# Benny44/QPALM

Hardware: AMD Instinct MI355X
Metric: QP solves/sec (batched random n=1000,m=2000); `value` = solve only, batch resident in HBM -- with qpalm_setup in the clock as the reference's run_time has it: `value_setup_plus_solve` (higher is better)
Workload: dtype f64

## Files before the change

qpalm_amd/csrc/qpalm_capi.inc:

```
#include <math.h>
#include <stdio.h>
#include <stdlib.h>
#include <string.h>
#include <sys/mman.h>

#include <algorithm>
#include <atomic>
#include <chrono>
#include <thread>
#include <string>
#include <vector>
#include <map>

#include "../../include/qpalm_gfx950.h"

#ifdef QP_TWO_INSTANCES
#define QP_INST(ns, kern) ns::kern
#else
#define QP_INST(ns, kern) kern
#define QP_T_SMALL QP_T
#define QP_LDS_SMALL 38912
#define QP_T_TINY QP_T
#define QP_LDS_TINY 22016
#define QP_TINY_PER_CU 7
// ... 39 lines not shown
  if (s->eps_abs_in < 0 || s->eps_rel_in < 0 || (s->eps_rel_in == 0 && s->eps_abs_in == 0)) return 0;
  if (s->rho <= 0 || s->rho >= 1) return 0;
  if (s->eps_prim_inf < 0 || s->eps_dual_inf < 0) return 0;
  if (s->theta > 1 || s->delta <= 1 || s->sigma_max <= 0) return 0;
  if (s->proximal != 0 && s->proximal != 1) return 0;
  if (s->gamma_init <= 0 || s->gamma_upd < 1 || s->gamma_max < s->gamma_init) return 0;
  if (s->scaling < 0) return 0;
  if (s->warm_start != 0 && s->warm_start != 1) return 0;
  if (s->verbose != 0 && s->verbose != 1) return 0;
  if (s->print_iter <= 0 || s->reset_newton_iter <= 0) return 0;
  if (s->enable_dual_termination != 0 && s->enable_dual_termination != 1) return 0;
  return 1;
}

static size_t align_up(size_t v, size_t a) { return (v + a - 1) / a * a; }

struct qpg_ctx {
  int device;
  int lds_bytes;
  int max_slots;
  int update_rank_threshold;
  int narrow_rows;
  int place_panel_wave;
  int small_workgroups;
  int coop;
  int coop_workgroups;
  int coop_max_batch;
  int coop_rank_threshold;
  int queue_order;
  int coop_test_kill;
  int coop_graphs;
  int coop_updates;
  int sweep_ranks;
  int factor_fused_solve;
  int kkt_compact;
  int sequential_rank_sums;
  int linesearch_hbm;
  int sparse_gpw;
  int sparse_lds;
  int sparse_ordering;
  int sparse_factor;
  int sparse_coop;
  int sparse_kkt;
  int ld_align;
  void *mv_buf[5];
  size_t mv_cap[5];
};

enum { H_AP, H_AI, H_ATP, H_ATI, H_ATPERM, H_AINV, H_QP, H_QI, H_QFP, H_QFI, H_QFPERM, H_AX, H_QX, H_Q, H_BMIN, H_BMAX, H_COUNT };
struct HostProblem {
  int n, m, nzA, nzQ, nzQf;
  double c;
  bool set;
};

struct qpg_batch {
  qpg_ctx *ctx;
  int B, n, m, nnzA, nnzQ, nnzQf, ld, nslots, ls_stride;
  int small, threads, lds_bytes;
  int kkt, nfac;
  QPGSettings settings;
  std::vector<HostProblem> probs;
  char *hslab; size_t hslab_bytes, hoff[H_COUNT + 1], hper[H_COUNT], helem[H_COUNT];
  template <class T> T *harr(int a, size_t b) const { return (T *)(hslab + hoff[a]) + b * hper[a]; }
  std::thread arena_thread; int arena_rc; bool arena_clean;
  std::vector<int> host_status;
// ... 10 lines not shown
  std::vector<SpPlan> sp_plan;
  qpg_view V;
  bool is_setup;
  float last_solve_ms;
  std::vector<std::pair<std::string, std::pair<void *, size_t> > > named;
  struct CoGraph { int uses; bool ready; rt_graph_t exec; };
  std::map<int, CoGraph> co_graphs;
  std::string co_sig;
  long co_replays;
  long co_sweeps;
  int nnzA_in, nnzQ_in;
  std::vector<std::vector<int> > map_A, map_Q;
  void *val_maps_d = nullptr; bool val_maps_current = false;
  std::vector<double> raw_h;
  void *raw_d = nullptr; int raw_cur = 0;
  double sens_floor = 0.0;
  double *raw_q() { return raw_h.data(); }
  double *raw_bmin() { return raw_h.data() + (size_t)B * n; }
  double *raw_bmax() { return raw_h.data() + (size_t)B * n + (size_t)B * m; }
  double *raw_d_q() const { return (double *)raw_d; }
  double *raw_d_bmin() const { return (double *)raw_d + (size_t)B * n; }
  double *raw_d_bmax() const { return (double *)raw_d + (size_t)B * n + (size_t)B * m; }
};
static void co_graphs_clear(qpg_batch *bt) {
  for (auto &g : bt->co_graphs) if (g.second.ready) RT_GRAPH_FREE(g.second.exec);
  bt->co_graphs.clear();
}

extern "C" int qpg_ctx_create(int device, qpg_ctx **out) {
  if (!out) return fail(QPG_ERR_INVALID, "qpg_ctx_create: out is NULL");
  std::string why;
  if (RT_DEVICE_INIT(device, why) != 0) return fail(QPG_ERR_NO_DEVICE, "qpg_ctx_create: " + why);
  qpg_ctx *c = new qpg_ctx();
  c->device = device; c->lds_bytes = QPG_LDS_DEFAULT; c->max_slots = 512; c->update_rank_threshold = -1; c->small_workgroups = 1; c->place_panel_wave = 0; c->narrow_rows = 1; c->coop = -1; c->coop_workgroups = 256; c->coop_max_batch = 4; c->coop_rank_threshold = -2; c->coop_updates = 2; c->coop_test_kill = 0; c->queue_order = 1; c->coop_graphs = 1; c->ld_align = 16; c->sweep_ranks = 16; c->kkt_compact = 1; c->factor_fused_solve = 1; c->sparse_factor = -1; c->sparse_kkt = 0; c->sparse_coop = 0; c->sparse_ordering = -1; c->sparse_lds = 1; c->sparse_gpw = 0; c->linesearch_hbm = 0; c->sequential_rank_sums = -1;
  for (int k = 0; k < 5; k++) { c->mv_buf[k] = nullptr; c->mv_cap[k] = 0; }
  *out = c;
  return api_ok();
}
extern "C" void qpg_ctx_destroy(qpg_ctx *ctx) {
  if (!ctx) return;
  for (int k = 0; k < 5; k++) if (ctx->mv_buf[k]) RT_FREE(ctx->mv_buf[k]);
  RT_RELEASE_STREAMS();
  delete ctx;
}
static int ctx_scratch(qpg_ctx *ctx, int k, size_t bytes, void **p) {
  if (bytes > ctx->mv_cap[k]) {
    if (ctx->mv_buf[k]) RT_FREE(ctx->mv_buf[k]);
    ctx->mv_buf[k] = nullptr; ctx->mv_cap[k] = 0;
    const size_t cap = align_up(bytes + bytes / 2, 4096);
    if (RT_MALLOC(&ctx->mv_buf[k], cap) != 0) return 1;
    ctx->mv_cap[k] = cap;
  }
  *p = ctx->mv_buf[k];
  return 0;
}
extern "C" int qpg_ctx_set_option(qpg_ctx *ctx, const char *name, qpg_int value) {
  if (!ctx || !name) return fail(QPG_ERR_INVALID, "qpg_ctx_set_option: NULL");
  if (!strcmp(name, "lds_bytes")) { if (value < QPG_LDS_DEFAULT || value > 160 * 1024 - 8192) return fail(QPG_ERR_INVALID, "lds_bytes out of range"); ctx->lds_bytes = (int)value; }
  else if (!strcmp(name, "max_slots")) { if (value < 1) return fail(QPG_ERR_INVALID, "max_slots < 1"); ctx->max_slots = (int)value; }
  else if (!strcmp(name, "update_rank_threshold")) ctx->update_rank_threshold = (int)value;
  else if (!strcmp(name, "small_workgroups")) ctx->small_workgroups = (value >= 0 && value <= 3) ? (int)value : 1;
  else if (!strcmp(name, "place_panel_wave")) ctx->place_panel_wave = (value < 0 || value > 2) ? 2 : (int)value;
  else if (!strcmp(name, "narrow_rows")) ctx->narrow_rows = value ? 1 : 0;
  else if (!strcmp(name, "coop")) ctx->coop = (value < 0) ? -1 : (value ? 1 : 0);
  else if (!strcmp(name, "coop_rank_threshold")) ctx->coop_rank_threshold = (value < -1) ? -2 : (int)value;
  else if (!strcmp(name, "coop_updates")) ctx->coop_updates = (value >= 0 && value <= 2) ? (int)value : 2;
  else if (!strcmp(name, "coop_graphs")) ctx->coop_graphs = value ? 1 : 0;
  else if (!strcmp(name, "coop_test_kill")) ctx->coop_test_kill = (int)value;
  else if (!strcmp(name, "queue_order")) ctx->queue_order = value ? 1 : 0;
  else if (!strcmp(name, "sweep_ranks")) { if (value != 16 && value != 32) return fail(QPG_ERR_INVALID, "sweep_ranks must be 16 or 32"); ctx->sweep_ranks = (int)value; }
  else if (!strcmp(name, "kkt_compact")) ctx->kkt_compact = value ? 1 : 0;
  else if (!strcmp(name, "factor_fused_solve")) ctx->factor_fused_solve = value ? 1 : 0;
  else if (!strcmp(name, "sparse_factor")) ctx->sparse_factor = (value < 0) ? -1 : (value ? 1 : 0);
  else if (!strcmp(name, "sparse_kkt")) ctx->sparse_kkt = value ? 1 : 0;
  else if (!strcmp(name, "sparse_coop")) { if (value != 0 && value != 1) return fail(QPG_ERR_INVALID, "sparse_coop must be 0 or 1"); ctx->sparse_coop = (int)value; }
  else if (!strcmp(name, "sequential_rank_sums")) ctx->sequential_rank_sums = (value < 0) ? -1 : (value ? 1 : 0);
  else if (!strcmp(name, "linesearch_hbm")) ctx->linesearch_hbm = (value < 0) ? 0 : (int)std::min<qpg_int>(value, 1 << 20);
  else if (!strcmp(name, "sparse_gpw")) ctx->sparse_gpw = (int)value;
  else if (!strcmp(name, "sparse_lds")) ctx->sparse_lds = (value < 0) ? 0 : (int)value;
  else if (!strcmp(name, "sparse_ordering")) ctx->sparse_ordering = (value < 0) ? -1 : (value ? 1 : 0);
  else if (!strcmp(name, "ld_align")) { if (value != 8 && value != 16 && value != 32) return fail(QPG_ERR_INVALID, "ld_align must be 8, 16 or 32"); ctx->ld_align = (int)value; }
  else if (!strcmp(name, "coop_max_batch")) { if (value < 1) return fail(QPG_ERR_INVALID, "coop_max_batch < 1"); ctx->coop_max_batch = (int)value; }
  else if (!strcmp(name, "coop_workgroups")) { if (value < 1 || value > 4096) return fail(QPG_ERR_INVALID, "coop_workgroups out of range"); ctx->coop_workgroups = (int)value; }
  else return fail(QPG_ERR_INVALID, std::string("unknown option ") + name);
  return api_ok();
}

static int arena_alloc(qpg_batch *bt);
static void *host_slab_alloc(size_t bytes) {
  void *p = mmap(nullptr, std::max<size_t>(bytes, 4096), PROT_READ | PROT_WRITE, MAP_PRIVATE | MAP_ANONYMOUS, -1, 0);
  if (p == MAP_FAILED) return nullptr;
#ifdef MADV_HUGEPAGE
  if (bytes >= ((size_t)64 << 20)) (void)madvise(p, bytes, MADV_HUGEPAGE);
#endif
  return p;
}
static void host_slab_free(void *p, size_t bytes) { if (p) munmap(p, std::max<size_t>(bytes, 4096)); }

extern "C" int qpg_batch_create(qpg_ctx *ctx, qpg_int B, qpg_int n, qpg_int m, qpg_int nnzA_max, qpg_int nnzQ_max,
                                const QPGSettings *settings, qpg_batch **out) {
  if (!ctx || !out) return fail(QPG_ERR_INVALID, "qpg_batch_create: NULL argument");
  if (B <= 0 || n <= 0 || m < 0 || nnzA_max < 0 || nnzQ_max < 0) return fail(QPG_ERR_INVALID, "qpg_batch_create: bad dimensions");
  if (!qpg_validate_settings(settings)) return fail(QPG_ERR_INVALID, "Settings validation returned failure");
// ... 696 lines not shown
  RT_MEMCPY_H2D(V.d, x0.data(), x0.size() * sizeof(double));
  BT_LAUNCH(bt, k_lobpcg, blocks_for(bt), 0, V);
  if (RT_SYNC() != 0) return fail(QPG_ERR_RUNTIME, "k_lobpcg failed: " + std::string(RT_LAST_ERROR()));
  return QPG_OK;
}

extern "C" int qpg_batch_setup(qpg_batch *bt) {
  if (!bt) return fail(QPG_ERR_INVALID, "qpg_batch_setup: NULL");
  for (int b = 0; b < bt->B; b++) if (!bt->probs[b].set) return fail(QPG_ERR_INVALID, "qpg_batch_setup: problem not set for every batch member");
  co_graphs_clear(bt);
  qpg_view &V = bt->V;
  if (bt->arena_thread.joinable()) bt->arena_thread.join();
  if (bt->arena_rc != 0 || !bt->arena_d) return fail(QPG_ERR_ALLOC, "device allocation failed");
  if (!bt->arena_clean) {
    RT_MEMSET(bt->arena_d, 0, bt->arena_d_bytes);
    if (RT_SYNC() != 0) return fail(QPG_ERR_RUNTIME, "arena clear failed: " + std::string(RT_LAST_ERROR()));
  }
  bt->arena_clean = false;
  bt->is_setup = false;
  bt->raw_h.clear(); bt->raw_cur = 0;
  bt->val_maps_current = false;
  V.B = bt->B; V.n = bt->n; V.m = bt->m; V.ld = bt->ld; V.nnzA = bt->nnzA; V.nnzQ = bt->nnzQ; V.nnzQf = bt->nnzQf;
  V.ls_hbm = bt->ctx->linesearch_hbm; V.seq_mode = bt->ctx->sequential_rank_sums;
  V.nslots = bt->nslots; V.lds_bytes = bt->lds_bytes; V.update_rank_threshold = bt->ctx->update_rank_threshold; V.place_panel_wave = bt->ctx->place_panel_wave;
  V.ls_stride = bt->ls_stride;
  {
    size_t nnz_rows = 0, rows = 0;
    for (auto &hp : bt->probs) { nnz_rows += (size_t)hp.nzA; rows += (size_t)hp.m; }
    const size_t colbufs = (size_t)4 * (bt->threads / 64) * bt->n * sizeof(double);
    V.narrow_rows = (bt->ctx->narrow_rows && !bt->kkt && colbufs <= (size_t)bt->lds_bytes && nnz_rows <= 16 * std::max<size_t>(rows, 1)) ? 1 : 0;
  }
  V.wst_stride = (int)QPG_WST_STRIDE(bt->nfac);
  V.sweep_ranks = bt->ctx->sweep_ranks;
  V.kkt_compact = bt->ctx->kkt_compact;
  V.factor_fused_solve = bt->ctx->factor_fused_solve;
  V.kkt = bt->kkt; V.nfac = bt->nfac;
  if (ensure_dual_slots(bt) != 0) return fail(QPG_ERR_ALLOC, "device allocation failed (LD_Q slots)");
  V.sparse = 0; V.sp_co_G = 0; V.sp_co_wv = nullptr;
  bt->sp_plan.clear();
  if (bt->sparse) {
    const int rcs = sparse_setup(bt);
    if (rcs != QPG_OK) return rcs;
    if (ensure_dual_slots(bt) != 0) return fail(QPG_ERR_ALLOC, "device allocation failed (LD_Q values of the sparse factor)");
  }
  const size_t B = bt->B, n = bt->n, m = bt->m;
  {
    char *const dev[H_COUNT] = {(char *)V.Ap, (char *)V.Ai, (char *)V.Atp, (char *)V.Ati, (char *)V.Atperm, (char *)V.Ainv, (char *)V.Qp, (char *)V.Qi,
                                (char *)V.Qfp, (char *)V.Qfi, (char *)V.Qfperm, (char *)V.Ax, (char *)V.Qx, (char *)V.q, (char *)V.bmin, (char *)V.bmax};
    for (int a = 0; a < H_COUNT; a++)
      if (bt->hper[a] && RT_MEMCPY_H2D_ASYNC(dev[a], bt->hslab + bt->hoff[a], B * bt->hper[a] * bt->helem[a], 0) != 0)
        return fail(QPG_ERR_RUNTIME, "upload failed: " + std::string(RT_LAST_ERROR()));
    RT_COPY_MARK(0);
    std::vector<double> c0(B);
    std::vector<qpg_scalars> sc(B);
    const qpg_scalars sc0 = setup_scalars(bt);
    for (size_t b = 0; b < B; b++) {
      c0[b] = bt->probs[b].c; sc[b] = sc0; bt->host_status[b] = QPG_UNSOLVED;
      const int *Qp = bt->harr<int>(H_QP, b), *Qi = bt->harr<int>(H_QI, b);
      const double *Qx = bt->harr<double>(H_QX, b);
      int hint = 0;
      for (int j = 0; j < bt->probs[b].n && !hint; j++) {
        bool pos = false;
        for (int k = Qp[j]; k < Qp[j + 1]; k++) if (Qi[k] == j && Qx[k] > 0.0) { pos = true; break; }
        if (!pos) hint = 1;
      }
      sc[b].seq_hint = hint;
// ... 1130 lines not shown
```

qpalm_amd/csrc/qpalm_dense.h:

```cpp
#ifndef QPALM_DENSE_H
#define QPALM_DENSE_H
#include <type_traits>

#ifdef QPALM_EMU
#define QP_FLAG_LOAD(p) (*(volatile int *)(p))
#define QP_FLAG_STORE(p, v) (*(volatile int *)(p) = (v))
#define QP_RELEASE_AGENT() do { } while (0)
#define QP_ACQUIRE_AGENT() do { } while (0)
#define QP_DRAIN_VMEM() do { } while (0)
#define QP_SLEEP() do { } while (0)
#define QP_WAVE_SYNC() emu_wave_sync()
#define QP_LDS_VBASE(p) (p)
#define QP_SCHED_BARRIER() do { } while (0)
#define QP_SETPRIO(p) do { } while (0)
#define QP_DRAIN_LDS() do { } while (0)
#else
#define QP_FLAG_LOAD(p) __hip_atomic_load((p), __ATOMIC_RELAXED, __HIP_MEMORY_SCOPE_AGENT)
#define QP_FLAG_STORE(p, v) __hip_atomic_store((p), (v), __ATOMIC_RELAXED, __HIP_MEMORY_SCOPE_AGENT)
#define QP_RELEASE_AGENT() __builtin_amdgcn_fence(__ATOMIC_RELEASE, "agent")
#define QP_ACQUIRE_AGENT() __builtin_amdgcn_fence(__ATOMIC_ACQUIRE, "agent")
#define QP_DRAIN_VMEM() asm volatile("s_waitcnt vmcnt(0)" ::: "memory")
#define QP_SLEEP() __builtin_amdgcn_s_sleep(2)
#define QP_SETPRIO(p) __builtin_amdgcn_s_setprio(p)
#define QP_DRAIN_LDS() asm volatile("s_waitcnt lgkmcnt(0)" ::: "memory")
// ... 953 lines not shown
  dnew = qp_rank_pivots_seq<KG>(p, ln, d0);
  const double sh = qp_row_shr<1>(dnew);
  dprev = ((ln & 15) == 0) ? d0 : sh;
  return (mode != QP_PIV_SEQ) ? 1 : 0;
}

#ifdef QPALM_EMU
template <int K, int OFF, int R0, int R1>
QPD void qp_apply_ranks_dpp(const double cw0, const double cw1, double (&wrow)[K], double &l) {
  const int lane = threadIdx.x & 63;
  emu_publish2(cw0, cw1);
  for (int r = R0; r < R1 && OFF + r < K; r++) {
    const double c0 = emu_peek((lane & ~15) | r, 0), c1 = emu_peek((lane & ~15) | r, 1);
    wrow[OFF + r] = QP_FMA(c0, l, wrow[OFF + r]);
    l = QP_FMA(c1, wrow[OFF + r], l);
  }
  emu_wave_sync();
}
#else
#define QP_FD_STEP(i, n) "v_fmac_f64_dpp %" #i ", %9, %8 row_newbcast:%" #n " row_mask:0xf bank_mask:0xf bound_ctrl:1\n\t" \
                         "v_fmac_f64_dpp %8, %10, %" #i " row_newbcast:%" #n " row_mask:0xf bank_mask:0xf bound_ctrl:1\n\t"
#define QP_FD_EIGHT QP_FD_STEP(0, 11) QP_FD_STEP(1, 12) QP_FD_STEP(2, 13) QP_FD_STEP(3, 14) QP_FD_STEP(4, 15) QP_FD_STEP(5, 16) QP_FD_STEP(6, 17) QP_FD_STEP(7, 18)
template <int R0> QPD void qp_fmac_bcast8(double *w, double &l, const double cw0, const double cw1) {
  asm("s_nop 1\n\t" QP_FD_EIGHT
      : "+&v"(w[0]), "+&v"(w[1]), "+&v"(w[2]), "+&v"(w[3]), "+&v"(w[4]), "+&v"(w[5]), "+&v"(w[6]), "+&v"(w[7]), "+&v"(l)
      : "v"(cw0), "v"(cw1), "n"(R0), "n"(R0 + 1), "n"(R0 + 2), "n"(R0 + 3), "n"(R0 + 4), "n"(R0 + 5), "n"(R0 + 6), "n"(R0 + 7));
}
template <int K, int OFF, int R0, int R1>
QPD void qp_apply_ranks_dpp(const double cw0, const double cw1, double (&wrow)[K], double &l) {
  static_assert(R1 - R0 == 8 && K % 8 == 0, "eight ranks at a time");
  if constexpr (OFF + R1 <= K) qp_fmac_bcast8<R0>(&wrow[OFF + R0], l, cw0, cw1);
}
#endif
#ifndef QP_AQD
#define QP_AQD 4
#endif

template <class IP, class DP, class WP>
QPD int updown_scatter_rows(const IP Atp, const IP Ati, const DP Atss, const int n, const WP Wst, const IP cols,
                            const int n_up, const IP cols_dn, const int r0, const int kk, const int lane, const int wid) {
  int jmin = n;
  for (int r = wid; r < kk; r += QP_NW) {
    const int g = r0 + r;
    const int t = (g < n_up) ? cols[g] : cols_dn[g - n_up];
    for (int k = Atp[t] + lane; k < Atp[t + 1]; k += 64) {
      const int i = Ati[k];
      Wst[(size_t)r * n + i] = Atss[k];
      jmin = (i < jmin) ? i : jmin;
    }
  }
  return jmin;
}

template <int RPT, int K>
QPNI void dense_updown(const int *Atp_, const int *Ati_, const double *Atss_, const int n_, const int ld_,
                       double *L_, double *Dg_, double *Wst_, const int *cols_, int n_up_,
                       const int *cols_dn_, int n_dn_, QpShared *S_, char *lds, int64_t *tdbg_, int pre_jmin_ = -1,
                       double *fs_ = nullptr, int rk0_ = 0, int rkn_ = 0x7fffffff) {
  const int n = QP_UNIFORM(n_), ld = QP_UNIFORM(ld_), n_up = QP_UNIFORM(n_up_), n_dn = QP_UNIFORM(n_dn_);
  const int rk0 = QP_UNIFORM(rk0_), rkn = QP_UNIFORM(rkn_);
  const int pre_jmin = QP_UNIFORM(pre_jmin_);
  const int pivmode = QP_UNIFORM(S_->seq_ranks);
  qp_gdouble *fs = (qp_gdouble *)fs_;
  const bool fuse_any = QP_UNIFORM((int)(fs_ != nullptr)) != 0;
  int64_t QP_LDS_AS *tdbg = (int64_t QP_LDS_AS *)tdbg_;
  const qp_gint *Atp = (const qp_gint *)Atp_, *Ati = (const qp_gint *)Ati_, *cols = (const qp_gint *)cols_, *cols_dn = (const qp_gint *)cols_dn_;
  const qp_gdouble *Atss = (const qp_gdouble *)Atss_;
  qp_gdouble *L = (qp_gdouble *)L_, *Dg = (qp_gdouble *)Dg_, *Wst = (qp_gdouble *)Wst_;
  QpShared &S = *S_;
  static_assert(K == 8 || K == 16 || K == 32, "rank groups of one DPP row (16 lanes), eight ranks at a time");
  static_assert(K <= QPG_KWST, "the staging area holds QPG_KWST dense update vectors");
  typedef UpdownLds<RPT, K> UpdownLdsT;
  UpdownLdsT QP_LDS_AS &U = *QP_LDS_ARG(UpdownLdsT, lds);
  static_assert(sizeof(UpdownLds<RPT, K>) <= ((RPT == 1) ? QP_LDS_BUDGET : QPG_LDS_DEFAULT), "update scratch must fit the dynamic LDS (the 256-thread instance only ever runs RPT = 1)");
  constexpr int NB = UpdownCfg<K>::NB, G = UpdownCfg<K>::G, KG = UpdownCfg<K>::KG;
  constexpr int PROWS = QP_T * RPT;
  constexpr bool MP = (K > 16);
  static_assert(PROWS % NB == 0, "passes start on block boundaries");
  const int lane = threadIdx.x & 63, wid = QP_UNIFORM(S.wave_rank[threadIdx.x >> 6]), tid = wid * 64 + lane;
  const int nr_all = n_up + n_dn;
  const int rk1 = (rkn < nr_all - rk0) ? (rk0 + rkn) : nr_all;
  qp_gdouble *dummy = Wst + (size_t)QPG_KWST * n;
  qp_gdouble *Tab = dummy + QPG_DUMMY + QPG_HSTASH;
  const int npass = MP ? (n + PROWS - 1) / PROWS : 1;
  for (int r0 = rk0; r0 < rk1; r0 += K) {
    const int kk = (rk1 - r0 < K) ? (rk1 - r0) : K;
    const bool fuse = fuse_any && (r0 + K >= nr_all);
    __syncthreads();
    long long tq0 = QP_CLOCK();
    int jmin = n;
    if (pre_jmin < 0) {
      for (int e = tid; e < kk * n; e += QP_T) Wst[e] = 0.0;
      __syncthreads();
      jmin = updown_scatter_rows(Atp, Ati, Atss, n, Wst, cols, n_up, cols_dn, r0, kk, lane, wid);
    } else jmin = (pre_jmin < n) ? pre_jmin : n - 1;
    if (fuse) jmin = 0;
    jmin = QP_UNIFORM(block_imin(S, jmin));
    double ialpha[G], sg[G];
    const int rl = lane & 15;
#pragma unroll
    for (int g = 0; g < G; g++) {
      ialpha[g] = 1.0;
      sg[g] = (16 * g + rl < kk) ? ((r0 + 16 * g + rl < n_up) ? 1.0 : -1.0) : 0.0;
    }
    const int J0 = (jmin / NB) * NB;
    if (tid == 0) {
      const long long tq1 = QP_CLOCK(); tdbg[0] += tq1 - tq0; tq0 = tq1;
      tdbg[QPG_CNT_SWEEPS] += 1;
      tdbg[QPG_CNT_SWEEP_ENTRIES] += (long long)(n - J0) * (n - J0 - 1) / 2 + (n - J0);
    }
    for (int pass = 0; pass < npass; pass++) {
    const int R0 = pass * PROWS;
    const int R1 = (!MP || n - R0 < PROWS) ? n : R0 + PROWS;
    const int Js = (J0 > R0) ? J0 : R0;
    if (Js >= R1) continue;
    const bool last_pass = (R1 >= n);
    const int rlim = last_pass ? ld : R1;
    if (MP && npass > 1) __syncthreads();
    double w[RPT][K];
#pragma unroll
// ... 156 lines not shown
      const bool own_live0 = (R0 + 64 * RPT - 1 >= Ja);
      auto owner_block = [&]() QP_ALWAYS_INLINE {
        const long long tt0 = QP_CLOCK();
        bool any = false;
#pragma unroll
        for (int rr = 0; rr < RPT; rr++) { const int i = R0 + tid * RPT + rr; any = any || (i >= Ja && i < R1); }
        constexpr bool WAVES = MP;
        if (s > 0 && (WAVES ? (__ballot(any ? 1 : 0) != 0ull) : any)) {
          const int i0 = R0 + tid * RPT;
          apply_table(prv, Jp, i0 >= Ja && i0 < rlim);
        }
#pragma unroll
        for (int rr = 0; rr < RPT; rr++) {
          const int i = R0 + tid * RPT + rr;
          if (i >= Jn && i < Jn + jbn) {
#pragma unroll
            for (int r = 0; r < K; r++) U.Wd[prv][i - Jn][r] = w[rr][r];
            U.Wd[prv][i - Jn][K] = acc[rr];
          }
        }
        if (wid == 0) {
#pragma unroll
          for (int rr = 0; rr < RPT; rr++)
#pragma unroll
            for (int r = 0; r < K; r++) U.stash[rr][r][lane] = w[rr][r];
#pragma unroll
          for (int rr = 0; rr < RPT; rr++) U.stash_acc[rr][lane] = acc[rr];
        }
        if (tid == QP_T - 64) tdbg[2] += QP_CLOCK() - tt0;
      };
      if (wid == 0) {
        const long long tp0 = QP_CLOCK();
        QP_SETPRIO(3);
        double wrow[K];
        double accp;
#pragma unroll
        for (int r = 0; r < K; r++) wrow[r] = (lane < jb) ? U.Wd[cur][lane][r] : 0.0;
        accp = (lane < jb) ? U.Wd[cur][lane][K] : 0.0;
        if (s > 0) {
          constexpr bool PSQ = QP_USQ;
          constexpr int QD = PSQ ? QP_AQD : 8;
          qp_gdouble *rowp = (lane < jb) ? (L + (size_t)Jp * ld + J + lane) : (dummy + lane);
          const size_t cstride = (lane < jb) ? (size_t)ld : 0;
          const int lrow = lane & (NB - 1);
          double q[QD];
#pragma unroll
          for (int cc = 0; cc < QD; cc++) q[cc] = PSQ ? U.Lsq[cur][cc][lrow] : rowp[(size_t)cc * cstride];
          const qp_pair QP_LDS_AS *tabA = (const qp_pair QP_LDS_AS *)QP_LDS_VBASE(&QP_CWG(U, prv, 0)[lane & 15][0]);
          constexpr bool PADPP = (K <= 16);
          qp_pair cfq[PADPP ? QD : 1][G];
          if (PADPP) {
#pragma unroll
            for (int cc = 0; cc < QD; cc++)
#pragma unroll
              for (int g = 0; g < G; g++) cfq[cc][g] = tabA[cc * K + 16 * g];
          }
          auto group = [&](const int c0) QP_ALWAYS_INLINE {
#pragma unroll
            for (int u = 0; u < QD; u++) {
              const int c1 = c0 + u;
              double l = q[u];
              const int cpre = (c1 + QD < NB) ? c1 + QD : NB - 1;
              if (PADPP) {
                qp_apply_ranks_dpp<K, 0, 0, 8>(cfq[u][0].x, cfq[u][0].y, wrow, l);
                if (KG > 8 && kk > 8) qp_apply_ranks_dpp<K, 0, 8, 16>(cfq[u][0].x, cfq[u][0].y, wrow, l);
                if constexpr (G > 1) {
// ... 62 lines not shown
              nwv[g] = 0.0; ngam[g] = 0.0;
              if (g > 0 && kkg <= 0) continue;
              const double wv = (rk < kkg) ? wt[(16 * g + rk) & (K - 1)] : 0.0;
              if (QP_PANEL_TIMING == 2 && g == 0) { QP_DRAIN_LDS(); const long long t = QP_CLOCK(); if (lane == 0) tdbg[8] += t - tc0; tc0 = t; }
              const double p = sg[g] * wv * wv * ialpha[g];
              double dnew, dprev;
              if (qp_rank_pivots<KG>(p, ln, d0, pivmode, dnew, dprev) && lane == 0) tdbg[QPG_CNT_SEQ_COLS] += 1;
              const double rdn = qp_rcp(dnew);
              const double gam = -sg[g] * wv * ialpha[g] * rdn;
              if (ln < KG) { QP_CWG(U, cur, c1)[16 * g + ln][0] = -wv; QP_CWG(U, cur, c1)[16 * g + ln][1] = -gam; }
              ialpha[g] = (wv == 0.0) ? ialpha[g] : ialpha[g] * dprev * rdn;
              d0 = qp_readlane(dnew, kkg - 1);
              nwv[g] = -wv; ngam[g] = -gam;
            }
            if (QP_PANEL_TIMING == 2) { double gg = ngam[0]; QP_OPAQUE_V(gg); const long long t = QP_CLOCK(); if (lane == 0) tdbg[9] += t - tc0; tc0 = t; }
            if (ln == c1) dreg = d0;
            double l = lcur;
            qp_apply_ranks_dpp<K, 0, 0, 8>(nwv[0], ngam[0], wrow, l);
            if (KG > 8 && kk > 8) qp_apply_ranks_dpp<K, 0, 8, 16>(nwv[0], ngam[0], wrow, l);
            if constexpr (G > 1) {
              if (kk > 16) qp_apply_ranks_dpp<K, 16, 0, 8>(nwv[1], ngam[1], wrow, l);
              if (kk > 24) qp_apply_ranks_dpp<K, 16, 8, 16>(nwv[1], ngam[1], wrow, l);
            }
            const bool below = (ln > c1 && ln < jb);
            if (below) U.Ld[cur][ln][c1] = l;
            if constexpr (FS) { const double yc = qp_readlane(vsub, c1); vsub = QP_FMA(-(below ? l : 0.0), yc, vsub); }
            if (QP_PANEL_TIMING == 2) { double ll = l; QP_OPAQUE_V(ll); const long long t = QP_CLOCK(); if (lane == 0) tdbg[11] += t - tc0; }
            QP_SCHED_BARRIER();
          }
        };
        if constexpr (FOLD) { if (fuse) recurrence(std::true_type()); else recurrence(std::false_type()); }
        else recurrence(std::false_type());
        if (QP_PANEL_TIMING == 1 && lane == 0) tdbg[9] += QP_CLOCK() - tp1;
        const long long tp2 = QP_CLOCK();
        if constexpr (!FOLD) if (fuse) {
          double lc = (lane > 0 && lane < jb) ? U.Ld[cur][lane][0] : 0.0;
#pragma unroll 1
          for (int c = 0; c < jb; c++) {
            const int ln = QP_FRESH_LANE(lane);
            const double lcn = (ln > c + 1 && ln < jb) ? U.Ld[cur][ln][c + 1] : 0.0;
            const double yc = qp_readlane(vsub, c);
            vsub = QP_FMA(-lc, yc, vsub);
            lc = lcn;
          }
        }
        if (fuse && lane < jb) { U.ys[cur][lane] = vsub; fs[J + lane] = vsub; }
        if (lane < jb) Dg[J + lane] = dreg;
        if (!QP_USQ) {
#pragma unroll 1
          for (int c = 0; c < jb; c++)
            if (lane > c && lane < jb) L[(size_t)(J + c) * ld + (J + lane)] = U.Ld[cur][lane][c];
        }
#pragma unroll
        for (int rr = 0; rr < RPT; rr++)
#pragma unroll
          for (int r = 0; r < K; r++) w[rr][r] = own_live0 ? U.stash[rr][r][lane] : 0.0;
#pragma unroll
        for (int rr = 0; rr < RPT; rr++) acc[rr] = own_live0 ? U.stash_acc[rr][lane] : 0.0;
        QP_SETPRIO(0);
        if (lane == 0) { tdbg[1] += QP_CLOCK() - tp0; tdbg[QPG_CNT_SWEEP_COLS] += jb; }
        if (QP_PANEL_TIMING == 1 && lane == 0) tdbg[10] += QP_CLOCK() - tp2;
        tpe = QP_CLOCK();
      }
      if (wid != 0 || own_live0) owner_block();
      constexpr int NFREE = (QP_NW == 1) ? 0 : 1;
      if (wid >= NFREE) {
        const int t0 = tid - 64 * NFREE, nt = QP_T - 64 * NFREE;
        if (QP_USQ) {
          for (int e = t0; e < NB * NB; e += nt) {
            const int c1 = e / NB, c = e % NB;
            if (c > c1) {
              if (s > 0) L[(size_t)(Jp + c1) * ld + (Jp + c)] = U.Ld[prv][c][c1];
              if (c < jbn) U.Ld[prv][c][c1] = L[(size_t)(Jn + c1) * ld + (Jn + c)];
            }
            if (jbn > 0) U.Lsq[prv][c1][c] = (c < jbn) ? L[(size_t)(J + c1) * ld + (Jn + c)] : 0.0;
          }
        } else {
          for (int e = t0; e < jbn * jbn; e += nt) {
            const int c1 = e / jbn, c = e % jbn;
            if (c > c1) U.Ld[prv][c][c1] = L[(size_t)(Jn + c1) * ld + (Jn + c)];
          }
        }
        if (t0 < jbn) U.dd[prv][t0] = Dg[Jn + t0];
        if (MP && !last_pass && s > 0) export_table(prv, Jp, t0, nt);
// ... 367 lines not shown
```

qpalm_amd/csrc/qpalm_device.h:

```cpp
#ifndef QPALM_DEVICE_H
#define QPALM_DEVICE_H

#include "qpalm_types.h"

#ifndef QP_T
#define QP_T 512
#endif
#define QP_NW (QP_T / 64)
#ifndef QP_KSEL
#define QP_KSEL(RPT) ((RPT) <= 2 ? 16 : 8)
#endif
#ifndef QP_K32
#ifdef QPALM_EMU
#define QP_K32(RPT) ((RPT) >= 1 && (RPT) <= 2)
#define QP_LDS_BUDGET QPG_LDS_DEFAULT
#else
#define QP_K32(RPT) (QP_T >= 512 && (RPT) >= 1 && (RPT) <= 2)
#define QP_LDS_BUDGET ((QP_T >= 512) ? QPG_LDS_DEFAULT : 38912)
#endif
#endif
#define QPD __device__ __forceinline__
#define QPN __device__ __forceinline__
#ifndef QP_PHASE_CALLS
#define QP_PHASE_CALLS 2
// ... 75 lines not shown
}
#define QP_FRESH_LANE(lane) qp_fresh_lane_()
static __device__ __forceinline__ int qp_fresh_tid_() {
  int t = (int)threadIdx.x;
  asm volatile("" : "+v"(t));
  return t & 1023;
}
#define QP_FRESH_TID() qp_fresh_tid_()
static __device__ __forceinline__ int qp_opaque_true_() {
  int one;
  asm volatile("s_mov_b32 %0, 1" : "=s"(one));
  return one;
}
#define QP_CALL_BLOCK() qp_opaque_true_()
#define QP_ALWAYS_INLINE __attribute__((always_inline))
#define QP_HW_SIMD() ((int)__builtin_amdgcn_s_getreg((2 - 1) << 11 | 4 << 6 | 4))
#define QP_HW_CU_KEY() ((int)(__builtin_amdgcn_s_getreg((8 - 1) << 11 | 8 << 6 | 4) | (__builtin_amdgcn_s_getreg((4 - 1) << 11 | 0 << 6 | 20) << 8)))
#endif

QPD double qmax(double a, double b) { return (a > b) ? a : b; }
QPD double qmin(double a, double b) { return (a < b) ? a : b; }
QPD double qabs(double x) { return (x < 0) ? -x : x; }

#define QP_NRED 20
struct QpShared {
  double red[QP_NW][QP_NRED];
  double bc[QP_NRED];
  int    ired[QP_NW][4];
  int    ibc[8];
  int    hw_simd[QP_NW];
  int    placement;
  int    panel_wave;
  int    seq_ranks;
  int    wave_rank[QP_NW];
};

#define QP_PIV_TREE 0
#define QP_PIV_SEQ 1
#define QP_PIV_GUARD 2
QPD int qp_pivot_mode(const qpg_view &V, int b) {
  if (V.seq_mode > 0 || (V.seq_mode < 0 && (V.sc[b].nc_flag != 0 || V.sc[b].seq_hint != 0))) return QP_PIV_SEQ;
  return (V.seq_mode < 0) ? QP_PIV_GUARD : QP_PIV_TREE;
}

QPD double wave_sum(double v) {
  for (int o = 32; o > 0; o >>= 1) v += __shfl_xor(v, o);
  return v;
}
QPD double wave_max(double v) {
  for (int o = 32; o > 0; o >>= 1) { double u = __shfl_xor(v, o); v = (u > v) ? u : v; }
  return v;
}
QPD int wave_isum(int v) {
  for (int o = 32; o > 0; o >>= 1) v += __shfl_xor(v, o);
  return v;
}
QPD int wave_imax(int v) {
  for (int o = 32; o > 0; o >>= 1) { int u = __shfl_xor(v, o); v = (u > v) ? u : v; }
  return v;
}
QPD int wave_imin(int v) {
  for (int o = 32; o > 0; o >>= 1) { int u = __shfl_xor(v, o); v = (u < v) ? u : v; }
  return v;
}

template <int NM, int NS>
// ... 148 lines not shown
```

qpalm_amd/csrc/qpalm_iter.h:

```cpp
#ifndef QPALM_ITER_H
#define QPALM_ITER_H
#ifndef QP_NOFUSE
#define QP_NOFUSE 0
#endif

#define QP_KIND_NEWTON 0
#define QP_KIND_OUTER 1
#define QP_KIND_FORCED 2
#define QP_KIND_TERMINATED 3

QPD int qp_prox(const qpg_settings &st, const qpg_scalars &s) { return (st.proximal != 0 || s.nc_flag != 0) ? 1 : 0; }
QPD double qp_gamma_init(const qpg_settings &st, const qpg_scalars &s) { return s.nc_flag ? s.nc_gamma : st.gamma_init; }
QPD double qp_gamma_max(const qpg_settings &st, const qpg_scalars &s) { return s.nc_flag ? s.nc_gamma : st.gamma_max; }

struct IterShared {
  QpShared S;
  qpg_scalars s;
  int kind, action, nL, pos;
  double a0, b0;
  double scan_a[QP_NW], scan_b[QP_NW];
};

struct QpArrays {
  const qpg_view *V; int b, n, m;
// ... 176 lines not shown
    }
  } else {
    for (int i = tid; i < m; i += QP_T) a.y()[i] = 0.;
  }
  __syncthreads();
  double vm[1] = {0.0}, vs[3] = {0.0, 0.0, 0.0};
  for (int j = tid; j < n; j += QP_T) { vs[0] += a.x()[j] * a.Qxv()[j]; vs[1] += a.q()[j] * a.x()[j]; }
  for (int i = tid; i < m; i += QP_T) {
    const double ax = a.Axv()[i];
    const double mid = qmax(a.bmin()[i], qmin(ax, a.bmax()[i]));
    const double t = ax + (-1) * mid;
    vs[2] += t * t;
  }
  block_reduce<0, 3>(I.S, vm, vs);
  const double f = 0.5 * vs[0] + vs[1], dist2 = vs[2];
  const double sig = qmax(1e-4, qmin(st.sigma_init * qmax(1, qabs(f)) / qmax(1, 0.5 * dist2), 1e4));
  const double ssig = QP_SQRT(sig), sinv = 1.0 / sig;
  for (int i = tid; i < m; i += QP_T) {
    a.sigma()[i] = sig; a.sigma_inv()[i] = sinv; a.sqrt_sigma()[i] = ssig; a.At_scale()[i] = ssig;
    for (int k = a.Atp()[i]; k < a.Atp()[i + 1]; k++) a.Atss()[k] = a.Atx()[k] * ssig;
  }
  if (tid == 0) { I.s.sqrt_sigma_max = QP_SQRT(st.sigma_max); I.s.initialized = 1; }
  __syncthreads();
}

template <int RPT>
QPN void dev_factor(const qpg_view &V, int n, double *L, double *Dg, char *lds, int64_t *tdbg, const double *fb = nullptr, double *fs = nullptr) { dense_factor(L, Dg, n, V.ld, lds, tdbg, fb, fs); }
template <int RPT>
QPN void dev_updown(const qpg_view &V, int b, int n, double *L, double *Dg, double *Wst, const int *up, int n_up,
                    const int *dn, int n_dn, QpShared &S, char *lds, int64_t *tdbg, double *fs = nullptr, int pre_jmin = -1) {
  const int *Atp = V.Atp + (size_t)b * (V.m + 1), *Ati = V.Ati + (size_t)b * V.nnzA;
  const double *Atss = V.Atss + (size_t)b * V.nnzA;
  __syncthreads();
  if (threadIdx.x == 0) S.seq_ranks = qp_pivot_mode(V, b);
  __syncthreads();
  if constexpr (RPT == 0) dense_updown_big<16>(Atp, Ati, Atss, n, V.ld, L, Dg, Wst, up, n_up, dn, n_dn, &S, lds, tdbg, pre_jmin);
  else if constexpr (QP_K32(RPT)) {
    const int nr = n_up + n_dn;
    int n32 = 0;
    if (V.sweep_ranks >= 32 && pre_jmin < 0 && nr > 16) n32 = (nr % 32 > 16 || nr % 32 == 0) ? nr : nr - nr % 32;
    if (n32 > 0) dense_updown<1, 32>(Atp, Ati, Atss, n, V.ld, L, Dg, Wst, up, n_up, dn, n_dn, &S, lds, tdbg, -1, (n32 == nr) ? fs : nullptr, 0, n32);
    if (n32 < nr) dense_updown<RPT, QP_KSEL(RPT)>(Atp, Ati, Atss, n, V.ld, L, Dg, Wst, up, n_up, dn, n_dn, &S, lds, tdbg, pre_jmin, fs, n32, nr - n32);
  } else dense_updown<RPT, QP_KSEL(RPT)>(Atp, Ati, Atss, n, V.ld, L, Dg, Wst, up, n_up, dn, n_dn, &S, lds, tdbg, pre_jmin, fs);
}

QPN void dev_ldlupdate_sigma_scale(const QpArrays &a, int nchg) {
  const int m = a.m, tid = threadIdx.x;
  __syncthreads();
  for (int k = tid; k < nchg; k += QP_T) {
    const int row = a.enter()[k];
    double s = a.At_scale()[row];
    s = s * s;
    s = QP_SQRT(1 - 1 / s);
    a.At_scale()[row] = s;
  }
  __syncthreads();
  for (int k = tid; k < m; k += QP_T) {
    const double s = a.At_scale()[k];
    if (s != 1.0) for (int e = a.Atp()[k]; e < a.Atp()[k + 1]; e++) a.Atss()[e] *= s;
  }
  __syncthreads();
}

QPD bool sp_update_pays(int nchange, int nlev, int n) { return (long long)nchange * (long long)nlev * 2 < (long long)n; }
QPP int dev_update_sigma_pre(const qpg_view &V, const QpArrays &a, IterShared &I) {
  const qpg_settings &st = *V.settings;
  const int n = a.n, m = a.m, tid = threadIdx.x;
// ... 823 lines not shown
```

qpalm_amd/csrc/qpalm_types.h:

```cpp
#ifndef QPALM_TYPES_H_GFX950
#define QPALM_TYPES_H_GFX950

#include <stdint.h>

#define QPG_SOLVED 1
#define QPG_DUAL_TERMINATED 2
#define QPG_MAX_ITER_REACHED (-2)
#define QPG_PRIMAL_INFEASIBLE (-3)
#define QPG_DUAL_INFEASIBLE (-4)
#define QPG_TIME_LIMIT_REACHED (-5)
#define QPG_UNSOLVED (-10)
#define QPG_ERROR 0
#define QPG_INFTY 1e20

typedef struct {
  int64_t max_iter, inner_max_iter;
  double eps_abs, eps_rel, eps_abs_in, eps_rel_in, rho, eps_prim_inf, eps_dual_inf, theta, delta, sigma_max,
      sigma_init;
  int64_t proximal;
  double gamma_init, gamma_upd, gamma_max;
  int64_t scaling, nonconvex, verbose, print_iter, warm_start, reset_newton_iter, enable_dual_termination;
  double dual_objective_limit, time_limit;
  int64_t ordering, factorization_method, max_rank_update;
  double max_rank_update_fraction;
// ... 6 lines not shown
#define QPG_CNT_FACTOR_REREAD 18
#define QPG_CNT_PLACEMENT 19
#define QPG_CNT_SEQ_COLS 20
#define QPG_CNT_SWEEP_COLS 21
#define QPG_LDS_DEFAULT 77824

typedef struct {
  double gamma, tau, eta, beta;
  double eps_pri, eps_dua, eps_dua_in, eps_abs_in, eps_rel_in, eps_k_abs, eps_k_rel;
  double sqrt_sigma_max, sqrt_delta, sc_c, sc_cinv;
  double pri_res_norm, dua_res_norm, dua2_res_norm, objective, dual_objective;
  double setup_time, solve_time;
  double nc_gamma, lobpcg_lambda, norm_Ax_z;
  int32_t nc_flag, lobpcg_iter;
  int32_t iter, iter_out, prev_iter, no_change;
  int32_t status, done, initialized, gamma_maxed, reset_newton, in_solve;
  int32_t nb_active, nb_enter, nb_leave, nb_sigma_changed;
  int32_t last_kind, last_fact, slot, has_scaling;
  int32_t pend_stage, pend_la, pend_action, pend_kind, pend_nchange;
  int32_t seq_hint;
  int32_t kkt_na;
  double pend_gam;
  int64_t pend_clock;
  int32_t guard_redo, n_guard_refactor, guard_spent, guard_pad;
  int32_t dual_pending, kkt_first;
  int32_t n_refactor, n_factor_Q, n_sweeps, n_rank1, n_solve, n_sigma_updates, n_boost_gamma, n_fused_solve;
  int64_t ticks_total, ticks_factor, ticks_update, ticks_solve, ticks_linesearch, ticks_resid;
  int64_t ticks_dbg[QPG_NDBG];
} qpg_scalars;

typedef struct {
  int32_t B, n, m, ld, nnzA, nnzQ, nnzQf, nslots, lds_bytes, update_rank_threshold, ls_stride, wst_stride, place_panel_wave, narrow_rows;
  int32_t offload, sweep_ranks;
  int32_t kkt_compact, factor_fused_solve;
  int32_t kkt, nfac;
  int32_t *Ap, *Ai, *Atp, *Ati, *Atperm, *Ainv, *Qp, *Qi, *Qfp, *Qfi, *Qfperm;
  double *Ax, *Atx, *Atss, *Qx, *Qfx;
  double *q, *bmin, *bmax, *c0;
  double *x, *y, *Axv, *Qxv, *Aty, *x_prev, *x0;
  double *sigma, *sigma_inv, *sqrt_sigma, *At_scale;
  double *Axys, *z, *pri_res, *pri_res_in, *yh, *Atyh, *df, *dphi, *dphi_prev, *d, *Qd, *Ad;
  double *delta_y, *delta_x, *temp_n, *temp_m;
  double *D, *Dinv, *E, *Einv;
  double *ls_key;
  int32_t *ls_idx;
  double *ls_delta, *ls_alpha;
  int32_t *active, *active_old, *enter, *leave;
  double *sol_x, *sol_y;
  double *L;
  double *Dg;
  double *LQ;
  double *DgQ;
  double *dual_rhs;
  double *kkt_sol, *kkt_rhs, *kkt_tmp, *kkt_rhs2;
  int32_t *nq, *mq;
  int32_t *kkt_list;
  int32_t *kkt_state;
  double *Wst;
  double *op_in, *op_out;
  int32_t sparse, sp_nnzL;
  int32_t *sp_Lp, *sp_Li;
  int32_t *sp_Rp, *sp_Rk, *sp_Rpos;
  int32_t *sp_levptr, *sp_levcol, *sp_nlev;
  double *sp_Lx;
  double *sp_wv;
  double *co_tab;
// ... 52 lines not shown
```

Baseline: 5797.

## Add short-chain panel kernel for low-rank (1,2,4) Cholesky updown sweeps

Adds a specialized panel routine for dense low-rank Cholesky up/downdates. When a rank group holds only 1, 2 or 4 ranks, it runs a shorter DPP broadcast FMA chain and a reduced pivot prefix scan instead of the full K-wide recurrence. This cuts the serial dependency length on the panel wave for the common small-rank updates. It is enabled by default through a new context option, adds code size and register pressure, and sends short cases through a separate numerical path.

```diff
diff --git a/qpalm_amd/csrc/qpalm_capi.inc b/qpalm_amd/csrc/qpalm_capi.inc
--- a/qpalm_amd/csrc/qpalm_capi.inc
+++ b/qpalm_amd/csrc/qpalm_capi.inc
@@ -95,6 +95,7 @@
   int coop_graphs;
   int coop_updates;
   int sweep_ranks;
+  int sweep_short_chain;
   int factor_fused_solve;
   int kkt_compact;
   int sequential_rank_sums;
@@ -171,7 +172,7 @@
   std::string why;
   if (RT_DEVICE_INIT(device, why) != 0) return fail(QPG_ERR_NO_DEVICE, "qpg_ctx_create: " + why);
   qpg_ctx *c = new qpg_ctx();
-  c->device = device; c->lds_bytes = QPG_LDS_DEFAULT; c->max_slots = 512; c->update_rank_threshold = -1; c->small_workgroups = 1; c->place_panel_wave = 0; c->narrow_rows = 1; c->coop = -1; c->coop_workgroups = 256; c->coop_max_batch = 4; c->coop_rank_threshold = -2; c->coop_updates = 2; c->coop_test_kill = 0; c->queue_order = 1; c->coop_graphs = 1; c->ld_align = 16; c->sweep_ranks = 16; c->kkt_compact = 1; c->factor_fused_solve = 1; c->sparse_factor = -1; c->sparse_kkt = 0; c->sparse_coop = 0; c->sparse_ordering = -1; c->sparse_lds = 1; c->sparse_gpw = 0; c->linesearch_hbm = 0; c->sequential_rank_sums = -1;
+  c->device = device; c->lds_bytes = QPG_LDS_DEFAULT; c->max_slots = 512; c->update_rank_threshold = -1; c->small_workgroups = 1; c->place_panel_wave = 0; c->narrow_rows = 1; c->coop = -1; c->coop_workgroups = 256; c->coop_max_batch = 4; c->coop_rank_threshold = -2; c->coop_updates = 2; c->coop_test_kill = 0; c->queue_order = 1; c->coop_graphs = 1; c->ld_align = 16; c->sweep_ranks = 16; c->sweep_short_chain = 1; c->kkt_compact = 1; c->factor_fused_solve = 1; c->sparse_factor = -1; c->sparse_kkt = 0; c->sparse_coop = 0; c->sparse_ordering = -1; c->sparse_lds = 1; c->sparse_gpw = 0; c->linesearch_hbm = 0; c->sequential_rank_sums = -1;
   for (int k = 0; k < 5; k++) { c->mv_buf[k] = nullptr; c->mv_cap[k] = 0; }
   *out = c;
   return api_ok();
@@ -208,6 +209,7 @@
   else if (!strcmp(name, "coop_test_kill")) ctx->coop_test_kill = (int)value;
   else if (!strcmp(name, "queue_order")) ctx->queue_order = value ? 1 : 0;
   else if (!strcmp(name, "sweep_ranks")) { if (value != 16 && value != 32) return fail(QPG_ERR_INVALID, "sweep_ranks must be 16 or 32"); ctx->sweep_ranks = (int)value; }
+  else if (!strcmp(name, "sweep_short_chain")) ctx->sweep_short_chain = value ? 1 : 0;
   else if (!strcmp(name, "kkt_compact")) ctx->kkt_compact = value ? 1 : 0;
   else if (!strcmp(name, "factor_fused_solve")) ctx->factor_fused_solve = value ? 1 : 0;
   else if (!strcmp(name, "sparse_factor")) ctx->sparse_factor = (value < 0) ? -1 : (value ? 1 : 0);
@@ -970,6 +972,7 @@
   }
   V.wst_stride = (int)QPG_WST_STRIDE(bt->nfac);
   V.sweep_ranks = bt->ctx->sweep_ranks;
+  V.sweep_short_chain = bt->ctx->sweep_short_chain;
   V.kkt_compact = bt->ctx->kkt_compact;
   V.factor_fused_solve = bt->ctx->factor_fused_solve;
   V.kkt = bt->kkt; V.nfac = bt->nfac;
diff --git a/qpalm_amd/csrc/qpalm_dense.h b/qpalm_amd/csrc/qpalm_dense.h
--- a/qpalm_amd/csrc/qpalm_dense.h
+++ b/qpalm_amd/csrc/qpalm_dense.h
@@ -1009,6 +1009,58 @@
   if constexpr (OFF + R1 <= K) qp_fmac_bcast8<R0>(&wrow[OFF + R0], l, cw0, cw1);
 }
 #endif
+
+#ifdef QPALM_EMU
+template <int KS> QPD void qp_apply_ranks_short(const double cw0, const double cw1, double *wrow, double &l) {
+  const int lane = threadIdx.x & 63;
+  emu_publish2(cw0, cw1);
+  for (int r = 0; r < KS; r++) {
+    const double c0 = emu_peek((lane & ~15) | r, 0), c1 = emu_peek((lane & ~15) | r, 1);
+    wrow[r] = QP_FMA(c0, l, wrow[r]);
+    l = QP_FMA(c1, wrow[r], l);
+  }
+  emu_wave_sync();
+}
+#else
+#define QP_FDS_STEP(w, l, c0, c1, n) "v_fmac_f64_dpp %" #w ", %" #c0 ", %" #l " row_newbcast:" #n " row_mask:0xf bank_mask:0xf bound_ctrl:1\n\t" \
+                                     "v_fmac_f64_dpp %" #l ", %" #c1 ", %" #w " row_newbcast:" #n " row_mask:0xf bank_mask:0xf bound_ctrl:1\n\t"
+QPD void qp_fmac_bcast1(double *w, double &l, const double cw0, const double cw1) {
+  asm("s_nop 1\n\t" QP_FDS_STEP(0, 1, 2, 3, 0) : "+&v"(w[0]), "+&v"(l) : "v"(cw0), "v"(cw1));
+}
+QPD void qp_fmac_bcast2(double *w, double &l, const double cw0, const double cw1) {
+  asm("s_nop 1\n\t" QP_FDS_STEP(0, 2, 3, 4, 0) QP_FDS_STEP(1, 2, 3, 4, 1) : "+&v"(w[0]), "+&v"(w[1]), "+&v"(l) : "v"(cw0), "v"(cw1));
+}
+QPD void qp_fmac_bcast4(double *w, double &l, const double cw0, const double cw1) {
+  asm("s_nop 1\n\t" QP_FDS_STEP(0, 4, 5, 6, 0) QP_FDS_STEP(1, 4, 5, 6, 1) QP_FDS_STEP(2, 4, 5, 6, 2) QP_FDS_STEP(3, 4, 5, 6, 3)
+      : "+&v"(w[0]), "+&v"(w[1]), "+&v"(w[2]), "+&v"(w[3]), "+&v"(l) : "v"(cw0), "v"(cw1));
+}
+template <int KS> QPD void qp_apply_ranks_short(const double cw0, const double cw1, double *wrow, double &l) {
+  static_assert(KS == 1 || KS == 2 || KS == 4, "one, two or four ranks");
+  if constexpr (KS == 1) qp_fmac_bcast1(&wrow[0], l, cw0, cw1);
+  else if constexpr (KS == 2) qp_fmac_bcast2(&wrow[0], l, cw0, cw1);
+  else qp_fmac_bcast4(&wrow[0], l, cw0, cw1);
+}
+#endif
+template <int KS, int KG> QPD int qp_rank_pivots_short(const double p, const int ln, const double d0, const int mode, double &dnew, double &dprev) {
+  if (mode != QP_PIV_SEQ) {
+    double incl = p;
+    if (KS > 1) incl += qp_row_shr<1>(incl);
+    if (KS > 2) { incl += qp_row_shr<2>(incl); incl += qp_row_shr<4>(incl); }
+    else incl += 0.0;
+    const double excl = qp_row_shr<1>(incl);
+    dnew = d0 + incl; dprev = d0 + excl;
+    if (mode == QP_PIV_TREE) return 0;
+    constexpr int NV = (KS > 2) ? ((KG > 8) ? 8 : 16) : KS;
+    bool danger = !(__builtin_fabs(dnew) >= 0x1p-8 * __builtin_fabs(d0));
+    if (KS == 2 && KG <= 8) danger = danger || !(__builtin_fabs(d0 + p) >= 0x1p-8 * __builtin_fabs(d0));
+    danger = danger && ((ln & 15) < NV);
+    if (__ballot(danger ? 1 : 0) == 0ull) return 0;
+  }
+  dnew = qp_rank_pivots_seq<KS>(p, ln, d0);
+  const double sh = qp_row_shr<1>(dnew);
+  dprev = ((ln & 15) == 0) ? d0 : sh;
+  return (mode != QP_PIV_SEQ) ? 1 : 0;
+}
 #ifndef QP_AQD
 #define QP_AQD 4
 #endif
@@ -1027,6 +1079,95 @@
     }
   }
   return jmin;
+}
+
+template <int RPT, int K, int KS>
+QPNI double updown_panel_short(char *lds, const int cur_, const int first_, const int jb_, const int kk_, const int pivmode_, const int fuse_,
+                               const double sg, double ialpha, double *L_, double *Dg_, double *fs_, double *dummy_, const int J_, const int ld_,
+                               int64_t *tdbg_) {
+  static_assert(K <= 16 && (KS == 1 || KS == 2 || KS == 4), "one rank group, short forms for 1, 2 and 4 ranks");
+  typedef UpdownLds<RPT, K> UpdownLdsT;
+  UpdownLdsT QP_LDS_AS &U = *QP_LDS_ARG(UpdownLdsT, lds);
+  constexpr int NB = UpdownCfg<K>::NB, KG = UpdownCfg<K>::KG;
+  const int cur = QP_UNIFORM(cur_), prv = cur ^ 1, jb = QP_UNIFORM(jb_), kk = QP_UNIFORM(kk_), pivmode = QP_UNIFORM(pivmode_);
+  const int J = QP_UNIFORM(J_), Jp = J - NB, ld = QP_UNIFORM(ld_);
+  const bool first = QP_UNIFORM(first_) != 0, fuse = QP_UNIFORM(fuse_) != 0;
+  qp_gdouble *L = (qp_gdouble *)L_, *Dg = (qp_gdouble *)Dg_, *fs = (qp_gdouble *)fs_, *dummy = (qp_gdouble *)dummy_;
+  int64_t QP_LDS_AS *tdbg = (int64_t QP_LDS_AS *)tdbg_;
+  const int lane = threadIdx.x & 63;
+  double wrow[KS];
+#pragma unroll
+  for (int r = 0; r < KS; r++) wrow[r] = (lane < jb) ? U.Wd[cur][lane][r] : 0.0;
+  double accp = (lane < jb) ? U.Wd[cur][lane][K] : 0.0;
+  if (!first) {
+    constexpr bool PSQ = QP_USQ, OWNA = QP_USQ;
+    constexpr int QD = PSQ ? QP_AQD : 8;
+    qp_gdouble *rowp = (lane < jb) ? (L + (size_t)Jp * ld + J + lane) : (dummy + lane);
+    const size_t cstride = (lane < jb) ? (size_t)ld : 0;
+    const int lrow = lane & (NB - 1);
+    double q[QD];
+#pragma unroll
+    for (int cc = 0; cc < QD; cc++) q[cc] = PSQ ? U.Lsq[cur][cc][lrow] : rowp[(size_t)cc * cstride];
+    const qp_pair QP_LDS_AS *tabA = (const qp_pair QP_LDS_AS *)QP_LDS_VBASE(&QP_CWG(U, prv, 0)[lane & 15][0]);
+    qp_pair cfq[QD];
+#pragma unroll
+    for (int cc = 0; cc < QD; cc++) cfq[cc] = tabA[cc * K];
+    auto group = [&](const int c0) QP_ALWAYS_INLINE {
+#pragma unroll
+      for (int u = 0; u < QD; u++) {
+        const int c1 = c0 + u;
+        double l = q[u];
+        const int cpre = (c1 + QD < NB) ? c1 + QD : NB - 1;
+        qp_apply_ranks_short<KS>(cfq[u].x, cfq[u].y, wrow, l);
+        if (!OWNA) rowp[(size_t)c1 * cstride] = l;
+        if (fuse) accp = QP_FMA(-l, U.ys[prv][c1], accp);
+        QP_SCHED_BARRIER();
+        q[u] = PSQ ? U.Lsq[cur][cpre][lrow] : rowp[(size_t)cpre * cstride];
+        cfq[u] = tabA[cpre * K];
+        QP_SCHED_BARRIER();
+      }
+    };
+    group(0);
+#pragma unroll 1
+    for (int c0 = QD; c0 < NB; c0 += QD) group(c0);
+  }
+  double dreg = (lane < jb) ? U.dd[cur][lane] : 1.0;
+  double lnext = (lane > 0 && lane < jb) ? U.Ld[cur][lane][0] : 0.0;
+  double vsub = accp;
+#pragma unroll 1
+  for (int c1 = 0; c1 < jb; c1++) {
+    const int ln = QP_FRESH_LANE(lane);
+    const double lcur = lnext;
+    lnext = (ln > c1 + 1 && ln < jb) ? U.Ld[cur][ln][c1 + 1] : 0.0;
+    const int rk = ln & 15;
+    const double d0 = qp_readlane(dreg, c1);
+    double wv = 0.0;
+#pragma unroll
+    for (int r = KS - 1; r >= 0; r--) { const double wr = qp_readlane(wrow[r], c1); wv = (rk == r) ? wr : wv; }
+    const double p = sg * wv * wv * ialpha;
+    double dnew, dprev;
+    if (qp_rank_pivots_short<KS, KG>(p, ln, d0, pivmode, dnew, dprev) && lane == 0) tdbg[QPG_CNT_SEQ_COLS] += 1;
+    const double rdn = qp_rcp(dnew);
+    const double gam = -sg * wv * ialpha * rdn;
+    if (ln < 4) { QP_CWG(U, cur, c1)[ln][0] = -wv; QP_CWG(U, cur, c1)[ln][1] = -gam; }
+    ialpha = (wv == 0.0) ? ialpha : ialpha * dprev * rdn;
+    const double dlast = qp_readlane(dnew, kk - 1);
+    if (ln == c1) dreg = dlast;
+    double l = lcur;
+    qp_apply_ranks_short<KS>(-wv, -gam, wrow, l);
+    const bool below = (ln > c1 && ln < jb);
+    if (below) U.Ld[cur][ln][c1] = l;
+    if (fuse) { const double yc = qp_readlane(vsub, c1); vsub = QP_FMA(-(below ? l : 0.0), yc, vsub); }
+    QP_SCHED_BARRIER();
+  }
+  if (fuse && lane < jb) { U.ys[cur][lane] = vsub; fs[J + lane] = vsub; }
+  if (lane < jb) Dg[J + lane] = dreg;
+  if (!QP_USQ) {
+#pragma unroll 1
+    for (int c = 0; c < jb; c++)
+      if (lane > c && lane < jb) L[(size_t)(J + c) * ld + (J + lane)] = U.Ld[cur][lane][c];
+  }
+  return ialpha;
 }
 
 template <int RPT, int K>
@@ -1063,6 +1204,12 @@
   for (int r0 = rk0; r0 < rk1; r0 += K) {
     const int kk = (rk1 - r0 < K) ? (rk1 - r0) : K;
     const bool fuse = fuse_any && (r0 + K >= nr_all);
+#ifdef QPALM_EMU
+    constexpr bool SHORT_OK = (K <= 16);
+#else
+    constexpr bool SHORT_OK = (K <= 16 && QP_T >= 512);
+#endif
+    const int ks = (SHORT_OK && QP_UNIFORM(S.short_chain) != 0) ? ((kk == 1) ? 1 : (kk == 2) ? 2 : (kk <= 4) ? 4 : 0) : 0;
     __syncthreads();
     long long tq0 = QP_CLOCK();
     int jmin = n;
@@ -1285,6 +1432,20 @@
       if (wid == 0) {
         const long long tp0 = QP_CLOCK();
         QP_SETPRIO(3);
+        long long tp2 = tp0;
+        bool general = true;
+        if constexpr (SHORT_OK) {
+          if (ks != 0) {
+            general = false;
+            char *const ul = (char *)&U; double *const Lg = (double *)L, *const Dgg = (double *)Dg, *const fsg = (double *)fs, *const dmy = (double *)dummy;
+            int64_t *const tg = (int64_t *)tdbg;
+            const int fi = (s == 0) ? 1 : 0, fu = fuse ? 1 : 0;
+            if (ks == 1) ialpha[0] = updown_panel_short<RPT, K, 1>(ul, cur, fi, jb, kk, pivmode, fu, sg[0], ialpha[0], Lg, Dgg, fsg, dmy, J, ld, tg);
+            else if (ks == 2) ialpha[0] = updown_panel_short<RPT, K, 2>(ul, cur, fi, jb, kk, pivmode, fu, sg[0], ialpha[0], Lg, Dgg, fsg, dmy, J, ld, tg);
+            else ialpha[0] = updown_panel_short<RPT, K, 4>(ul, cur, fi, jb, kk, pivmode, fu, sg[0], ialpha[0], Lg, Dgg, fsg, dmy, J, ld, tg);
+          }
+        }
+        if (general) {
         double wrow[K];
         double accp;
 #pragma unroll
@@ -1413,7 +1574,7 @@
         if constexpr (FOLD) { if (fuse) recurrence(std::true_type()); else recurrence(std::false_type()); }
         else recurrence(std::false_type());
         if (QP_PANEL_TIMING == 1 && lane == 0) tdbg[9] += QP_CLOCK() - tp1;
-        const long long tp2 = QP_CLOCK();
+        tp2 = QP_CLOCK();
         if constexpr (!FOLD) if (fuse) {
           double lc = (lane > 0 && lane < jb) ? U.Ld[cur][lane][0] : 0.0;
 #pragma unroll 1
@@ -1431,6 +1592,7 @@
 #pragma unroll 1
           for (int c = 0; c < jb; c++)
             if (lane > c && lane < jb) L[(size_t)(J + c) * ld + (J + lane)] = U.Ld[cur][lane][c];
+        }
         }
 #pragma unroll
         for (int rr = 0; rr < RPT; rr++)
diff --git a/qpalm_amd/csrc/qpalm_device.h b/qpalm_amd/csrc/qpalm_device.h
--- a/qpalm_amd/csrc/qpalm_device.h
+++ b/qpalm_amd/csrc/qpalm_device.h
@@ -131,6 +131,7 @@
   int    placement;
   int    panel_wave;
   int    seq_ranks;
+  int    short_chain;
   int    wave_rank[QP_NW];
 };
 
diff --git a/qpalm_amd/csrc/qpalm_iter.h b/qpalm_amd/csrc/qpalm_iter.h
--- a/qpalm_amd/csrc/qpalm_iter.h
+++ b/qpalm_amd/csrc/qpalm_iter.h
@@ -232,7 +232,7 @@
   const int *Atp = V.Atp + (size_t)b * (V.m + 1), *Ati = V.Ati + (size_t)b * V.nnzA;
   const double *Atss = V.Atss + (size_t)b * V.nnzA;
   __syncthreads();
-  if (threadIdx.x == 0) S.seq_ranks = qp_pivot_mode(V, b);
+  if (threadIdx.x == 0) { S.seq_ranks = qp_pivot_mode(V, b); S.short_chain = V.sweep_short_chain; }
   __syncthreads();
   if constexpr (RPT == 0) dense_updown_big<16>(Atp, Ati, Atss, n, V.ld, L, Dg, Wst, up, n_up, dn, n_dn, &S, lds, tdbg, pre_jmin);
   else if constexpr (QP_K32(RPT)) {
diff --git a/qpalm_amd/csrc/qpalm_types.h b/qpalm_amd/csrc/qpalm_types.h
--- a/qpalm_amd/csrc/qpalm_types.h
+++ b/qpalm_amd/csrc/qpalm_types.h
@@ -62,6 +62,7 @@
 typedef struct {
   int32_t B, n, m, ld, nnzA, nnzQ, nnzQf, nslots, lds_bytes, update_rank_threshold, ls_stride, wst_stride, place_panel_wave, narrow_rows;
   int32_t offload, sweep_ranks;
+  int32_t sweep_short_chain;
   int32_t kkt_compact, factor_fused_solve;
   int32_t kkt, nfac;
   int32_t *Ap, *Ai, *Atp, *Ati, *Atperm, *Ainv, *Qp, *Qi, *Qfp, *Qfi, *Qfperm;
```

Measured after the change: 5855, median of 6. About the same (+1.0%).
